# GaodeRender/triangle-splatting

Hardware: AMD Instinct MI355X
Metric: fwd+bwd Mpixels/sec @ 1M triangles, 1920x1080; achieved HBM GB/s (higher is better)
Workload: dtype f32

## Files before the change

triangle-splatting_amd/csrc/api.hip:

```cpp
#pragma GCC visibility push(default)
#include "../../include/ts2d.h"
#ifdef TS2D_LAB
#include "ts2d_lab.h"
#endif
#pragma GCC visibility pop
#include "ts2d_api.h"
#include <atomic>
#include <chrono>
#include <cstdarg>
#include <cstdio>
#include <cstring>
#include <mutex>
#include <string>
#include <vector>

namespace
{
thread_local std::string g_err;

struct ProfRow { std::string name; double ms = 0; int64_t launches = 0; };
struct ProfPending { int row; hipEvent_t a, b; };
std::mutex g_prof_mu;
bool g_prof_on = false;
std::string g_prof_only;
// ... 621 lines not shown
    case 8: src = g.tiles_touched; bytes = (size_t)P * 4; break;
    case 9:
    {
        std::vector<uint2> rc((size_t)P);
        if (dst_bytes < (size_t)P * 16) return ts_fail(TS2D_ERR_CAPACITY, "dst too small");
        if (P > 0)
        {
            TS_HIP(hipMemcpyAsync(rc.data(), g.rect, (size_t)P * sizeof(uint2), hipMemcpyDeviceToHost, s));
            TS_HIP(hipStreamSynchronize(s));
        }
        uint32_t *o = (uint32_t *)dst;
        for (int i = 0; i < P; i++)
        {
            o[4 * i] = rc[i].x & 0xffffu; o[4 * i + 1] = rc[i].x >> 16;
            o[4 * i + 2] = rc[i].y & 0xffffu; o[4 * i + 3] = rc[i].y >> 16;
        }
        return TS2D_OK;
    }
    case 10:
    {
        if (dst_bytes < (size_t)N * 8) return ts_fail(TS2D_ERR_CAPACITY, "dst too small");
        std::vector<uint32_t> tile((size_t)N), vals((size_t)N), depth((size_t)P);
        if (N > 0)
        {
            TS_HIP(hipMemcpyAsync(tile.data(), b.tile, (size_t)N * 4, hipMemcpyDeviceToHost, s));
            TS_HIP(hipMemcpyAsync(vals.data(), b.vals, (size_t)N * 4, hipMemcpyDeviceToHost, s));
            TS_HIP(hipMemcpyAsync(depth.data(), g.depth, (size_t)P * 4, hipMemcpyDeviceToHost, s));
            TS_HIP(hipStreamSynchronize(s));
        }
        uint64_t *o = (uint64_t *)dst;
        const uint32_t keymask = ts_tile_keymask(gx * gy);
        for (int64_t i = 0; i < N; i++) o[i] = ((uint64_t)(tile[i] & keymask) << 32) | depth[vals[i] & TS_ID_MASK];
        return TS2D_OK;
    }
    case 11: src = b.vals; bytes = (size_t)N * 4; break;
    case 12: src = im.ranges; bytes = (size_t)gx * gy * 8; break;
    case 13: src = im.n_contrib; bytes = (size_t)W * H * 4; break;
    case 14: src = im.final_T; bytes = (size_t)W * H * 4; break;
    case 15: src = b.k[(b.passes & 1) ^ 1]; bytes = (size_t)N * 4; break;
    case 16: src = b.v[(b.passes & 1) ^ 1]; bytes = (size_t)N * 4; break;
    case 17:
    {
        uint32_t top_const = 0;
        if (P > 0)
        {
            TS_HIP(hipMemcpyAsync(&top_const, g.top_const, 4, hipMemcpyDeviceToHost, s));
            TS_HIP(hipStreamSynchronize(s));
        }
        src = top_const ? g.sv[0] : g.sv[1];
        bytes = (size_t)P * 4;
        break;
    }
    case 18: src = g.rec; bytes = (size_t)P * TS_REC_FLOATS * 4; break;
    default: return ts_fail(TS2D_ERR_INVALID, "unknown field %d", field);
    }
    if (dst_bytes < bytes) return ts_fail(TS2D_ERR_CAPACITY, "dst too small");
    if (bytes)
    {
        TS_HIP(hipMemcpyAsync(dst, src, bytes, hipMemcpyDeviceToHost, s));
        TS_HIP(hipStreamSynchronize(s));
    }
    return TS2D_OK;
}

void ts2d_lab_force_ticket_passes(int on) { ts_force_ticket_passes(on != 0); }
void ts2d_lab_force_all_quadrants(int on) { g_lab_all_quadrants = on != 0; }
void ts2d_lab_force_kernel_cull(int on) { g_lab_kernel_cull = on != 0; }
void ts2d_lab_force_depth_pass4(int on) { ts_force_depth_pass4(on != 0); }
void ts2d_lab_depth_split(int mode, int bucket_cap) { ts_lab_depth_split(mode, bucket_cap); }
#endif

void ts2d_profile_enable(int on)
{
    std::lock_guard<std::mutex> lk(g_prof_mu);
    g_prof_on = on != 0;
}
void ts2d_profile_only(const char *name)
{
    std::lock_guard<std::mutex> lk(g_prof_mu);
    g_prof_only = name ? name : "";
}
void ts2d_profile_reset(void)
{
    std::lock_guard<std::mutex> lk(g_prof_mu);
    prof_drain();
    g_prof_rows.clear();
}
int ts2d_profile_read(int32_t index, char *name, size_t name_bytes, double *total_ms, int64_t *launches)
{
    std::lock_guard<std::mutex> lk(g_prof_mu);
    prof_drain();
    if (index < 0 || (size_t)index >= g_prof_rows.size()) return TS2D_ERR_INVALID;
    const ProfRow &r = g_prof_rows[index];
    if (name && name_bytes) { strncpy(name, r.name.c_str(), name_bytes - 1); name[name_bytes - 1] = 0; }
    if (total_ms) *total_ms = r.ms;
    if (launches) *launches = r.launches;
    return TS2D_OK;
}
}
```

triangle-splatting_amd/csrc/emit.hip:

```cpp
#include "ts2d_radix.h"
#include "ts2d_support.h"

namespace
{
constexpr uint32_t SMALL = 32;

#ifndef TS_EMIT_WAVES
#define TS_EMIT_WAVES 6
#endif
template <bool BM>
#if TS_EMIT_WAVES > 0
__global__ void __launch_bounds__(256, TS_EMIT_WAVES) scan_emit_kernel(
#else
__global__ void __launch_bounds__(256) scan_emit_kernel(
#endif
int P, int grid_x, int ntiles, GeometryStateView g, BinningStateView b, uint2 *ranges,
                                                         float *contrib_sum, float *contrib_max, long long capacity, int32_t *status, bool two_level,
                                                         QuadMaskArgs qmask)
{
    __shared__ uint32_t wtot[4];
    __shared__ unsigned long long wpart[4];
    const int t = threadIdx.x, lane = t & 63, wave = t >> 6;
    const int i = blockIdx.x * 256 + t;
    for (int k = i; k < ntiles; k += gridDim.x * 256) ranges[k] = make_uint2(0u, 0u);
    if (b.rs.tickets)
    {
        for (int k = i; k < b.rs.slabs + TS_RS_TICKET_EXTRA; k += gridDim.x * 256) b.rs.tickets[k] = 0u;
        for (int k = i; k < b.rs.slabs * NB; k += gridDim.x * 256) b.rs.slabacc[0][k] = 0u;
    }
    if (contrib_sum && i < P)
    {
        contrib_sum[i] = 0.0f;
        contrib_max[i] = 0.0f;
    }
    const bool valid = i < P;
    uint32_t tiles = valid ? g.tiles_sorted[i] : 0u;
    const uint32_t id_ahead = valid ? sorted_ids(g)[i] : 0u;
    const int sblock = blockIdx.x >> 2, quarter = blockIdx.x & 3;
    unsigned long long part = 0;
    if (two_level)
    {
        for (int k = t; k < (sblock >> 6); k += 256) part += g.supersum[k];
        if (t < (sblock & 63)) part += g.blocksum[(sblock & ~63) + t];
    }
    else
        for (int k = t; k < sblock; k += 256) part += g.blocksum[k];
    for (int q = 0; q < quarter; q++)
    {
        const int j = (sblock * 4 + q) * 256 + t;
        part += (j < P) ? g.tiles_sorted[j] : 0u;
    }
    if (capacity >= 0)
    {
        const unsigned long long live = g.blocksum[(P + SB - 1) / SB];
        const bool over = live > (unsigned long long)capacity;
        if (i == 0 && status) *status = over ? 1 : 0;
        if (over) tiles = 0u;
    }
    else if (i == 0 && status) *status = 0;
    const uint32_t inc = wave_inclusive_scan(tiles, lane);
    for (int o = 32; o > 0; o >>= 1) part += __shfl_xor(part, o);
    if (lane == 63) wtot[wave] = inc;
    if (lane == 0) wpart[wave] = part;
    __syncthreads();
    uint32_t before = 0;
    for (int w = 0; w < wave; w++) before += wtot[w];
    const unsigned long long qbase = wpart[0] + wpart[1] + wpart[2] + wpart[3];
    const uint32_t incl = (uint32_t)(qbase + before + inc);
    if (valid) g.offsets[i] = incl;
    const uint32_t id = tiles > 0 ? id_ahead : 0u;
    const uint32_t off = incl - tiles;
    uint2 rect = {0u, 0u};
    float4 rec0 = make_float4(0, 0, 0, 0), rec1 = rec0, rec2 = rec0;
    if (tiles > 0)
    {
        rect = g.rect[id];
        const float4 *rp = g.rec + 4 * (size_t)id;
        rec0 = rp[0];
        rec1 = rp[1];
        if (qmask.variant == 3) rec2 = rp[2];
    }
    const uint32_t minx = rect.x & 0xffffu, miny = rect.x >> 16, maxx = rect.y & 0xffffu, maxy = rect.y >> 16;
    uint32_t *tile_out = b.k[0], *val_out = b.v[0];
    constexpr bool qm = true;
    constexpr bool bm = BM;
    const float quad_g2 = qmask.g2;
    auto setup_from = [&](const float4 &r0, const float4 &r1, const float4 &r2, uint32_t tminx, uint32_t tminy, uint32_t tmaxx, uint32_t tmaxy) {
        if (qmask.variant == 0) return quad_setup_all();
        if (qmask.variant == 3)
        {
            const float E = quad_g2 == 2.0f ? support_scale<true>(1.0f, quad_g2) : support_scale<false>(1.0f, quad_g2);
            return quad_setup_3d(r0, r1, r2, E, qmask.tan_fovx, qmask.tan_fovy, qmask.W, qmask.H, qmask.inv_W, qmask.inv_H, (float)(tminx * TS_TILE) - 1.0f,
                                 (float)(tminy * TS_TILE) - 1.0f, (float)(tmaxx * TS_TILE), (float)(tmaxy * TS_TILE));
        }
        const float E = quad_g2 == 2.0f ? support_scale<true>(r1.z, quad_g2) : support_scale<false>(r1.z, quad_g2);
        return quad_setup<bm ? 3 : 7>(r0.x, r0.y, r0.z, r0.w, r1.x, r1.y, E);
    };
    auto setup_of = [&](uint32_t tri, uint32_t tminx, uint32_t tminy, uint32_t tmaxx, uint32_t tmaxy) {
        const float4 *rp = g.rec + 4 * (size_t)tri;
        return setup_from(rp[0], rp[1], qmask.variant == 3 ? rp[2] : make_float4(0, 0, 0, 0), tminx, tminy, tmaxx, tmaxy);
    };
    QuadSetup qs{};
    constexpr uint32_t STAGE = 2048;
    __shared__ uint32_t stage_t[STAGE];
    __shared__ __attribute__((aligned(16))) float4 region_b[256 * 4];
    uint32_t *const stage_v = (uint32_t *)region_b;
    const uint32_t run0 = (uint32_t)qbase, run = wtot[0] + wtot[1] + wtot[2] + wtot[3];
    const bool staged = run <= STAGE;
    const bool qstage = qm && staged;
    const uint32_t rw = maxx - minx, rh = maxy - miny;
    if (qm && tiles > 0)
    {
        qs = setup_from(rec0, rec1, rec2, minx, miny, maxx, maxy);
        if (qstage)
        {
            const QuadAffine qa = quad_anchor(qs, id, minx, miny, rw, rh);
            region_b[4 * t] = qa.a; region_b[4 * t + 1] = qa.b; region_b[4 * t + 2] = qa.c; region_b[4 * t + 3] = qa.d;
        }
    }
    if (tiles > 0 && tiles <= SMALL)
    {
        uint32_t o = off;
        if (staged)
        {
            o -= run0;
            for (uint32_t y = miny; y < maxy; y++)
                for (uint32_t x = minx; x < maxx; x++)
                {
                    stage_t[o] = qstage ? ((x - minx) | ((y - miny) << 12) | ((uint32_t)t << 24)) : y * grid_x + x;
                    if (!qstage) stage_v[o] = id;
                    o++;
                }
        }
        else
            for (uint32_t y = miny; y < maxy; y++)
                for (uint32_t x = minx; x < maxx; x++)
                {
                    if (bm)
                    {
                        const uint32_t m16 = block_mask(qs, (float)(x * TS_TILE), (float)(y * TS_TILE));
                        tile_out[o] = (y * grid_x + x) | (m16 << 16);
                        val_out[o] = id | (quadrants_of_blocks(m16) << TS_ID_BITS);
                    }
                    else
                    {
                        tile_out[o] = y * grid_x + x;
                        val_out[o] = qm ? id | (quadrant_mask(qs, (float)(x * TS_TILE), (float)(y * TS_TILE)) << TS_ID_BITS) : id;
                    }
                    o++;
                }
    }
    unsigned long long big = ballot64(tiles > SMALL);
    while (big)
    {
        const int j = __builtin_ctzll(big);
        big &= big - 1;
        const uint32_t t_minx = __shfl(minx, j), t_miny = __shfl(miny, j), t_maxx = __shfl(maxx, j), t_maxy = __shfl(maxy, j);
        const uint32_t t_tiles = __shfl(tiles, j), t_off = __shfl(off, j), t_id = __shfl(id, j);
        const uint32_t w = t_maxx - t_minx;
        QuadSetup tq{};
        if (qm && !staged) tq = setup_of(t_id, t_minx, t_miny, t_maxx, t_maxy);
        for (uint32_t k = lane; k < t_tiles; k += 64)
        {
            const uint32_t y = t_miny + k / w, x = t_minx + k % w;
            if (staged)
            {
                stage_t[t_off - run0 + k] = qstage ? ((k % w) | ((k / w) << 12) | ((uint32_t)(wave * 64 + j) << 24)) : y * grid_x + x;
                if (!qstage) stage_v[t_off - run0 + k] = t_id;
            }
            else
            {
                if (bm)
                {
                    const uint32_t m16 = block_mask(tq, (float)(x * TS_TILE), (float)(y * TS_TILE));
                    tile_out[t_off + k] = (y * grid_x + x) | (m16 << 16);
                    val_out[t_off + k] = t_id | (quadrants_of_blocks(m16) << TS_ID_BITS);
                }
                else
                {
                    tile_out[t_off + k] = y * grid_x + x;
                    val_out[t_off + k] = qm ? t_id | (quadrant_mask(tq, (float)(x * TS_TILE), (float)(y * TS_TILE)) << TS_ID_BITS) : t_id;
                }
            }
        }
    }
    if (staged)
    {
        __syncthreads();
        for (uint32_t k = t; k < run; k += 256)
        {
            uint32_t tl = stage_t[k], v;
            if (qstage)
            {
                const uint32_t dx = tl & 0xfffu, dy = (tl >> 12) & 0xfffu, slot = tl >> 24;
                QuadAffine qa;
                qa.a = region_b[4 * slot]; qa.b = region_b[4 * slot + 1]; qa.c = region_b[4 * slot + 2]; qa.d = region_b[4 * slot + 3];
                const uint32_t org = __float_as_uint(qa.d.z), x = (org & 0xffffu) + dx, y = (org >> 16) + dy;
                if (bm)
                {
                    const uint32_t m16 = block_mask_affine(qa, dx, dy, x, y);
                    v = __float_as_uint(qa.d.y) | (quadrants_of_blocks(m16) << TS_ID_BITS);
                    tl = (y * grid_x + x) | (m16 << 16);
                }
                else
                {
                    v = __float_as_uint(qa.d.y) | (quadrant_mask_affine(qa, dx, dy, x, y) << TS_ID_BITS);
                    tl = y * grid_x + x;
                }
            }
            else v = stage_v[k];
            tile_out[run0 + k] = tl;
            val_out[run0 + k] = v;
        }
    }
}

__global__ void __launch_bounds__(256) tile_ranges_kernel(int64_t N, const unsigned long long *n_dev, const uint32_t *__restrict__ tile,
                                                           uint2 *__restrict__ ranges, uint32_t keymask)
{
    const int64_t i0 = ((int64_t)blockIdx.x * 256 + threadIdx.x) * 4;
    if (n_dev)
    {
        const unsigned long long live = *n_dev;
        N = (live <= (unsigned long long)N) ? (int64_t)live : 0;
    }
    if (i0 >= N) return;
    uint32_t k[4];
    if (i0 + 3 < N)
    {
        const uint4 q = *(const uint4 *)(tile + i0);
        k[0] = q.x & keymask; k[1] = q.y & keymask; k[2] = q.z & keymask; k[3] = q.w & keymask;
    }
    else
        for (int j = 0; j < 4; j++) k[j] = i0 + j < N ? tile[i0 + j] & keymask : 0u;
    uint32_t prev = i0 > 0 ? tile[i0 - 1] & keymask : 0u;
#pragma unroll
    for (int j = 0; j < 4; j++)
    {
        const int64_t i = i0 + j;
        if (i >= N) break;
        const uint32_t cur = k[j];
        if (i == 0) ranges[cur].x = 0;
        else if (cur != prev)
        {
            ranges[prev].y = (uint32_t)i;
            ranges[cur].x = (uint32_t)i;
        }
        if (i == N - 1) ranges[cur].y = (uint32_t)N;
        prev = cur;
    }
}
}

void ts_launch_emit_keys(int P, int grid_x, int ntiles, const GeometryStateView &g, const BinningStateView &b, const ImageStateView &im,
                         float *contrib_sum, float *contrib_max, int64_t capacity, int32_t *status, const QuadMaskArgs &qmask, hipStream_t s)
{
    if (P <= 0) return;
    const dim3 grid((unsigned)(((P + SB - 1) / SB) * 4));
    if (qmask.blocks)
        hipLaunchKernelGGL(scan_emit_kernel<true>, grid, dim3(256), 0, s, P, grid_x, ntiles, g, b, im.ranges, contrib_sum, contrib_max, (long long)capacity,
                           status, ts_scan_two_level(P), qmask);
    else
        hipLaunchKernelGGL(scan_emit_kernel<false>, grid, dim3(256), 0, s, P, grid_x, ntiles, g, b, im.ranges, contrib_sum, contrib_max, (long long)capacity,
                           status, ts_scan_two_level(P), qmask);
}
const unsigned long long *ts_instance_count_dev(const GeometryStateView &g, int P) { return (const unsigned long long *)(g.blocksum + (P + SB - 1) / SB); }

void ts_launch_tile_ranges(int64_t N, const unsigned long long *n_dev, int ntiles, const BinningStateView &b, const ImageStateView &im, hipStream_t s)
{
    if (N <= 0) return;
    hipLaunchKernelGGL(tile_ranges_kernel, dim3((unsigned)((N + 1023) / 1024)), dim3(256), 0, s, N, n_dev, b.tile, im.ranges, ts_tile_keymask(ntiles));
}
```

triangle-splatting_amd/csrc/mesh_preprocess.hip:

```cpp
#include "ts2d_common.h"
#include "ts2d_math.h"
#include "ts2d_preprocess_launch.h"

using namespace ts;

namespace
{
constexpr float BOX_MARGIN = 2e-3f;

__global__ void __launch_bounds__(256) mesh_preprocess_kernel(MeshArgs a, GeometryStateView g)
{
    const int f = blockIdx.x * 256 + threadIdx.x;
    clear_tickets(g, f, a.F);
    if (f >= a.F) return;
    uint32_t out_tiles = 0;
    uint2 out_rect = {0u, 0u};
    float out_key = 0.0f;
    float rec[TS_REC_FLOATS];
#pragma unroll
    for (int i = 0; i < TS_REC_FLOATS; i++) rec[i] = 0.0f;

    int32_t i1 = a.faces[3 * (size_t)f], i2 = a.faces[3 * (size_t)f + 1], i3 = a.faces[3 * (size_t)f + 2];
    if (i1 > i2) { const int32_t t = i1; i1 = i2; i2 = t; }
    if (i2 > i3) { const int32_t t = i2; i2 = i3; i3 = t; }
    if (i1 > i2) { const int32_t t = i1; i1 = i2; i2 = t; }
    do
    {
        if ((uint32_t)i1 >= (uint32_t)a.V || (uint32_t)i2 >= (uint32_t)a.V || (uint32_t)i3 >= (uint32_t)a.V) break;
        const float *p1 = a.vertices + 3 * (size_t)i1, *p2 = a.vertices + 3 * (size_t)i2, *p3 = a.vertices + 3 * (size_t)i3;
        const f3 v1 = xform_point_4x3({p1[0], p1[1], p1[2]}, a.viewmatrix), v2 = xform_point_4x3({p2[0], p2[1], p2[2]}, a.viewmatrix),
                 v3 = xform_point_4x3({p3[0], p3[1], p3[2]}, a.viewmatrix);
        if (!(v1.z > a.znear && v2.z > a.znear && v3.z > a.znear)) break;

        const float hw = (float)a.W * 0.5f, hh = (float)a.H * 0.5f;
        const f2 s1 = {(v1.x / (v1.z * a.tan_fovx) + 1.0f) * hw, (v1.y / (v1.z * a.tan_fovy) + 1.0f) * hh};
        const f2 s2 = {(v2.x / (v2.z * a.tan_fovx) + 1.0f) * hw, (v2.y / (v2.z * a.tan_fovy) + 1.0f) * hh};
        const f2 s3 = {(v3.x / (v3.z * a.tan_fovx) + 1.0f) * hw, (v3.y / (v3.z * a.tan_fovy) + 1.0f) * hh};
        const float area2 = cross(sub(s2, s1), sub(s3, s1));
        if (!(fabsf(area2) > 0.0f)) break;

        const float xmin = fminf(fminf(s1.x, s2.x), s3.x), xmax = fmaxf(fmaxf(s1.x, s2.x), s3.x);
        const float ymin = fminf(fminf(s1.y, s2.y), s3.y), ymax = fmaxf(fmaxf(s1.y, s2.y), s3.y);
        if (!(xmax >= 0.0f && xmin <= (float)a.W && ymax >= 0.0f && ymin <= (float)a.H)) break;
        const int px0 = max(0, f2i(ceilf(fmaxf(xmin, 0.0f) - 0.5f - BOX_MARGIN))), px1 = min(a.W - 1, f2i(floorf(fminf(xmax, (float)a.W) - 0.5f + BOX_MARGIN)));
        const int py0 = max(0, f2i(ceilf(fmaxf(ymin, 0.0f) - 0.5f - BOX_MARGIN))), py1 = min(a.H - 1, f2i(floorf(fminf(ymax, (float)a.H) - 0.5f + BOX_MARGIN)));
        if (px1 < px0 || py1 < py0) break;
        const int rminx = px0 / TS_TILE, rminy = py0 / TS_TILE, rmaxx = px1 / TS_TILE + 1, rmaxy = py1 / TS_TILE + 1;

        const f3 n = cross(sub(v2, v1), sub(v3, v1));
        rec[0] = s1.x; rec[1] = s1.y; rec[2] = s2.x; rec[3] = s2.y; rec[4] = s3.x; rec[5] = s3.y;
        rec[6] = n.x; rec[7] = n.y; rec[8] = n.z;
        rec[9] = dot(n, v1);
        rec[10] = fminf(fminf(v1.z, v2.z), v3.z);
        rec[11] = fmaxf(fmaxf(v1.z, v2.z), v3.z);
        out_key = rec[10];
        out_tiles = (uint32_t)(rmaxx - rminx) * (uint32_t)(rmaxy - rminy);
        out_rect = {(uint32_t)rminx | ((uint32_t)rminy << 16), (uint32_t)rmaxx | ((uint32_t)rmaxy << 16)};
    } while (false);

    g.tiles_touched[f] = out_tiles;
    g.rect[f] = out_rect;
    g.depth[f] = out_key;
    float4 *r = g.rec + 4 * (size_t)f;
    r[0] = make_float4(rec[0], rec[1], rec[2], rec[3]);
    r[1] = make_float4(rec[4], rec[5], rec[6], rec[7]);
    r[2] = make_float4(rec[8], rec[9], rec[10], rec[11]);
    r[3] = make_float4(rec[12], rec[13], rec[14], rec[15]);
}
}

void ts_launch_mesh_preprocess(const MeshArgs &a, const GeometryStateView &g, hipStream_t s)
{
    if (a.F <= 0) return;
    hipLaunchKernelGGL(mesh_preprocess_kernel, dim3((unsigned)((a.F + 255) / 256)), dim3(256), 0, s, a, g);
}
```

triangle-splatting_amd/csrc/preprocess.hip:

```cpp
#include "ts2d_common.h"
#include "ts2d_math.h"
#include "ts2d_sh.h"
#include "ts2d_preprocess_launch.h"

using namespace ts;

namespace
{
__device__ __forceinline__ void preprocess_fwd_one(const PreprocessArgs &a, int32_t *__restrict__ radii, const GeometryStateView &g,
                                                   int idx, const float *vp, const float *shp, float4 *rec_row)
{
    int out_radius = 0;
    uint32_t out_tiles = 0;
    uint2 out_rect = {0u, 0u};
    uint8_t out_clamped = 0;
    float out_depth = 0.0f;
    float rec[TS_REC_FLOATS];
#pragma unroll
    for (int i = 0; i < TS_REC_FLOATS; i++) rec[i] = 0.0f;

    const f3 v1 = {vp[0], vp[1], vp[2]}, v2 = {vp[3], vp[4], vp[5]}, v3 = {vp[6], vp[7], vp[8]};
    const f3 center = divf(add(add(v1, v2), v3), 3.0f);
    const f3 center_proj = project_point(center, a.projmatrix);

// ... 30 lines not shown
        if (a.back_culling) { if (area2 >= -TS_EPS) break; }
        else { if (fabsf(area2) < TS_EPS) break; }

        const float dilation = 3.0f;
        const f2 d1 = add(center_2D, scale(dilation, r1_2D));
        const f2 d2 = add(center_2D, scale(dilation, r2_2D));
        const f2 d3 = add(center_2D, scale(dilation, r3_2D));
        const f2 v_min = {fminf(fminf(d1.x, d2.x), d3.x), fminf(fminf(d1.y, d2.y), d3.y)};
        const f2 v_max = {fmaxf(fmaxf(d1.x, d2.x), d3.x), fmaxf(fmaxf(d1.y, d2.y), d3.y)};

        const int rminx = min(a.grid_x, max(0, f2i(v_min.x / TS_TILE)));
        const int rminy = min(a.grid_y, max(0, f2i(v_min.y / TS_TILE)));
        const int rmaxx = min(a.grid_x, max(0, f2i((v_max.x + TS_TILE - 1) / TS_TILE)));
        const int rmaxy = min(a.grid_y, max(0, f2i((v_max.y + TS_TILE - 1) / TS_TILE)));
        if (rmaxx <= rminx || rmaxy <= rminy) break;

        {
        f3 rgb = {0, 0, 0};
        if (a.use_shs)
        {
            const f3 cp = {a.campos[0], a.campos[1], a.campos[2]};
            rgb = sh_to_rgb(a.D, shp, center, cp);
            out_clamped = (uint8_t)((rgb.x < 0 ? 1 : 0) | (rgb.y < 0 ? 2 : 0) | (rgb.z < 0 ? 4 : 0));
            rgb = {fmaxf(rgb.x, 0.0f), fmaxf(rgb.y, 0.0f), fmaxf(rgb.z, 0.0f)};
        }
        else
        {
            const float *fp = a.feature + (size_t)idx * a.C;
            rgb.x = a.C > 0 ? fp[0] : 0.0f;
            rgb.y = a.C > 1 ? fp[1] : 0.0f;
            rgb.z = a.C > 2 ? fp[2] : 0.0f;
        }
        rec[0] = v1_2D.x; rec[1] = v1_2D.y; rec[2] = v2_2D.x; rec[3] = v2_2D.y; rec[4] = v3_2D.x; rec[5] = v3_2D.y;
        rec[6] = a.opacity[idx];
        rec[7] = rgb.x; rec[8] = rgb.y; rec[9] = rgb.z;
        if (a.rich_info)
        {
            f3 n_view = cross(r1_view, r2_view);
            n_view = divf(n_view, norm(n_view));
            rec[10] = n_view.x; rec[11] = n_view.y; rec[12] = n_view.z;
            rec[13] = r1_view.z + center_view.z; rec[14] = r2_view.z + center_view.z; rec[15] = r3_view.z + center_view.z;
        }
        }
        out_depth = center_view.z;
        out_tiles = (uint32_t)(rmaxx - rminx) * (uint32_t)(rmaxy - rminy);
        out_rect = {(uint32_t)rminx | ((uint32_t)rminy << 16), (uint32_t)rmaxx | ((uint32_t)rmaxy << 16)};
        out_radius = f2i(fmaxf(ceilf((v_max.x - v_min.x) * 0.5f), ceilf((v_max.y - v_min.y) * 0.5f)));
    } while (false);

    {
        radii[idx] = out_radius;
        g.tiles_touched[idx] = out_tiles;
        g.rect[idx] = out_rect;
        g.depth[idx] = out_depth;
        g.clamped[idx] = out_clamped;
        float4 *r = rec_row;
        r[0] = make_float4(rec[0], rec[1], rec[2], rec[3]);
        r[1] = make_float4(rec[4], rec[5], rec[6], rec[7]);
        r[2] = make_float4(rec[8], rec[9], rec[10], rec[11]);
        r[3] = make_float4(rec[12], rec[13], rec[14], rec[15]);
    }
}

__device__ __forceinline__ void project_vec_approx_bwd(f3 p, f3 v, float tx, float ty, f2 dL_dvec_proj, f3 &dL_dp, f3 &dL_dv)
{
    const float px_pz = p.x / p.z, py_pz = p.y / p.z;
    const float vx_pz = v.x / p.z, vy_pz = v.y / p.z, vz_pz = v.z / p.z;
    const f2 d = {dL_dvec_proj.x / (p.z * tx), dL_dvec_proj.y / (p.z * ty)};
    dL_dv = {d.x, d.y, -d.x * px_pz - d.y * py_pz};
    dL_dp = {-d.x * vz_pz, -d.y * vz_pz, d.x * (2.0f * vz_pz * px_pz - vx_pz) + d.y * (2.0f * vz_pz * py_pz - vy_pz)};
}

__device__ __forceinline__ void preprocess_bwd_one(const PreprocessArgs &a, const int32_t *__restrict__ radii,
                                                   const GeometryStateView &g, const float *__restrict__ grad_rec, int idx,
                                                   const float *vp, const float *shp, float *ov, float *osh,
                                                   float *__restrict__ dL_dcenter2D, float *__restrict__ dL_dfeature,
                                                   float *__restrict__ dL_dopacity)
{
    float *oc = dL_dcenter2D + 2 * (size_t)idx;
    if (radii[idx] <= 0)
    {
#pragma unroll
        for (int i = 0; i < 9; i++) ov[i] = 0.0f;
        oc[0] = 0.0f; oc[1] = 0.0f;
        dL_dopacity[idx] = 0.0f;
        for (int c = 0; c < a.C; c++) dL_dfeature[(size_t)idx * a.C + c] = 0.0f;
        if (a.use_shs && osh)
        {
#pragma unroll
            for (int k = 0; k < 48; k++)
                if (k < a.M * 3) osh[k] = 0.0f;
        }
        return;
    }

    const float4 *gr = (const float4 *)(grad_rec + TS_GRAD_FLOATS * (size_t)idx);
    const float4 g0 = gr[0], g1 = gr[1], g2 = gr[2], g3 = gr[3];
    const f2 dL_dv1_2D = {g0.x, g0.y}, dL_dv2_2D = {g0.z, g0.w}, dL_dv3_2D = {g1.x, g1.y};
    const float dL_dop = g1.z;
    f3 dL_drgb = {g1.w, g2.x, g2.y};
    const f3 dL_dnormal_view = {g2.z, g2.w, g3.x};
    const f3 dL_dv_depth = {g3.y, g3.z, g3.w};

    const f3 v1 = {vp[0], vp[1], vp[2]}, v2 = {vp[3], vp[4], vp[5]}, v3 = {vp[6], vp[7], vp[8]};
    const f3 center = divf(add(add(v1, v2), v3), 3.0f);
    const f3 center_view = xform_point_4x3(center, a.viewmatrix);
// ... 102 lines not shown
```

triangle-splatting_amd/csrc/preprocess3d.hip:

```cpp
#include "ts2d_common.h"
#include "ts2d_math.h"
#include "ts2d_sh.h"
#include "ts2d_preprocess_launch.h"

using namespace ts;

namespace
{
__device__ __forceinline__ float proj_to_pix(float v, int S) { return (v + 1.0f) * S * 0.5f - 0.5f; }

__device__ __forceinline__ void preprocess3d_fwd_one(const PreprocessArgs &a, int32_t *__restrict__ radii, const GeometryStateView &g,
                                                     int idx, const float *vp, const float *shp, float4 *rec_row)
{
    int out_radius = 0;
    uint32_t out_tiles = 0;
    uint2 out_rect = {0u, 0u};
    uint8_t out_clamped = 0;
    float out_depth = 0.0f;
    float rec[TS_REC_FLOATS];
#pragma unroll
    for (int i = 0; i < TS_REC_FLOATS; i++) rec[i] = 0.0f;

    const f3 v1 = {vp[0], vp[1], vp[2]}, v2 = {vp[3], vp[4], vp[5]}, v3 = {vp[6], vp[7], vp[8]};
    do
// ... 5 lines not shown
        if (norm(normal_view) < TS_EPS) break;
        if (a.back_culling && normal_view.z >= 0) break;

        const float dilation = 3.0f;
        const f3 center = divf(add(add(v1, v2), v3), 3.0f);
        const f3 d1 = add(center, scale(dilation, sub(v1, center)));
        const f3 d2 = add(center, scale(dilation, sub(v2, center)));
        const f3 d3 = add(center, scale(dilation, sub(v3, center)));
        const f3 p1 = project_point(d1, a.projmatrix), p2 = project_point(d2, a.projmatrix), p3 = project_point(d3, a.projmatrix);
        if (p1.z <= 0 || p2.z <= 0 || p3.z <= 0) break;

        const f2 q1 = {proj_to_pix(p1.x, a.W), proj_to_pix(p1.y, a.H)};
        const f2 q2 = {proj_to_pix(p2.x, a.W), proj_to_pix(p2.y, a.H)};
        const f2 q3 = {proj_to_pix(p3.x, a.W), proj_to_pix(p3.y, a.H)};
        const f2 v_min = {fminf(fminf(q1.x, q2.x), q3.x), fminf(fminf(q1.y, q2.y), q3.y)};
        const f2 v_max = {fmaxf(fmaxf(q1.x, q2.x), q3.x), fmaxf(fmaxf(q1.y, q2.y), q3.y)};
        const int rminx = min(a.grid_x, max(0, f2i(v_min.x / TS_TILE)));
        const int rminy = min(a.grid_y, max(0, f2i(v_min.y / TS_TILE)));
        const int rmaxx = min(a.grid_x, max(0, f2i((v_max.x + TS_TILE - 1) / TS_TILE)));
        const int rmaxy = min(a.grid_y, max(0, f2i((v_max.y + TS_TILE - 1) / TS_TILE)));
        if (rmaxx <= rminx || rmaxy <= rminy) break;

        f3 rgb = {0, 0, 0};
        if (a.use_shs)
        {
            const f3 cp = {a.campos[0], a.campos[1], a.campos[2]};
            rgb = sh_to_rgb(a.D, shp, center, cp);
            out_clamped = (uint8_t)((rgb.x < 0 ? 1 : 0) | (rgb.y < 0 ? 2 : 0) | (rgb.z < 0 ? 4 : 0));
            rgb = {fmaxf(rgb.x, 0.0f), fmaxf(rgb.y, 0.0f), fmaxf(rgb.z, 0.0f)};
        }
        else
        {
            const float *fp = a.feature + (size_t)idx * a.C;
            rgb.x = a.C > 0 ? fp[0] : 0.0f;
            rgb.y = a.C > 1 ? fp[1] : 0.0f;
            rgb.z = a.C > 2 ? fp[2] : 0.0f;
        }
        rec[0] = v1_view.x; rec[1] = v1_view.y; rec[2] = v1_view.z;
        rec[3] = v2_view.x; rec[4] = v2_view.y; rec[5] = v2_view.z;
        rec[6] = v3_view.x; rec[7] = v3_view.y; rec[8] = v3_view.z;
        rec[9] = normal_view.x; rec[10] = normal_view.y; rec[11] = normal_view.z;
        rec[12] = a.opacity[idx];
        rec[13] = rgb.x; rec[14] = rgb.y; rec[15] = rgb.z;
        out_depth = center_view.z;
        out_tiles = (uint32_t)(rmaxx - rminx) * (uint32_t)(rmaxy - rminy);
        out_rect = {(uint32_t)rminx | ((uint32_t)rminy << 16), (uint32_t)rmaxx | ((uint32_t)rmaxy << 16)};
        out_radius = f2i(fmaxf(ceilf((v_max.x - v_min.x) * 0.5f), ceilf((v_max.y - v_min.y) * 0.5f)));
    } while (false);

    {
        radii[idx] = out_radius;
        g.tiles_touched[idx] = out_tiles;
        g.rect[idx] = out_rect;
        g.depth[idx] = out_depth;
        g.clamped[idx] = out_clamped;
        float4 *r = rec_row;
        r[0] = make_float4(rec[0], rec[1], rec[2], rec[3]);
        r[1] = make_float4(rec[4], rec[5], rec[6], rec[7]);
        r[2] = make_float4(rec[8], rec[9], rec[10], rec[11]);
        r[3] = make_float4(rec[12], rec[13], rec[14], rec[15]);
    }
}

__device__ __forceinline__ void preprocess3d_bwd_one(const PreprocessArgs &a, const int32_t *__restrict__ radii,
                                                     const GeometryStateView &g, const float *__restrict__ grad_rec, int idx,
                                                     const float *vp, const float *shp, float *ov, float *osh,
                                                     float *__restrict__ dL_dcenter2D, float *__restrict__ dL_dfeature,
                                                     float *__restrict__ dL_dopacity)
{
    float *oc = dL_dcenter2D + 2 * (size_t)idx;
    if (radii[idx] <= 0)
    {
#pragma unroll
        for (int i = 0; i < 9; i++) ov[i] = 0.0f;
        oc[0] = 0.0f; oc[1] = 0.0f;
        dL_dopacity[idx] = 0.0f;
        for (int c = 0; c < a.C; c++) dL_dfeature[(size_t)idx * a.C + c] = 0.0f;
        if (a.use_shs && osh)
        {
#pragma unroll
            for (int k = 0; k < 48; k++)
                if (k < a.M * 3) osh[k] = 0.0f;
        }
        return;
    }
    const f3 v1 = {vp[0], vp[1], vp[2]}, v2 = {vp[3], vp[4], vp[5]}, v3 = {vp[6], vp[7], vp[8]};
    const float4 *rp = g.rec + 4 * (size_t)idx;
    const float4 r0 = rp[0], r1 = rp[1], r2 = rp[2];
    const f3 v1_view = {r0.x, r0.y, r0.z}, v2_view = {r0.w, r1.x, r1.y}, v3_view = {r1.z, r1.w, r2.x};
    const float4 *gr = (const float4 *)(grad_rec + TS_GRAD_FLOATS * (size_t)idx);
    const float4 g0 = gr[0], g1 = gr[1], g2 = gr[2], g3 = gr[3];
    f3 gv1 = {g0.x, g0.y, g0.z}, gv2 = {g0.w, g1.x, g1.y}, gv3 = {g1.z, g1.w, g2.x};
    const f3 gn = {g2.y, g2.z, g2.w};
    const float gop = g3.x;
    const f3 grgb = {g3.y, g3.z, g3.w};
    f3 grgb_out = grgb;

    gv1 = add(gv1, cross(sub(v2_view, v3_view), gn));
    gv2 = add(gv2, cross(sub(v3_view, v1_view), gn));
    gv3 = add(gv3, cross(sub(v1_view, v2_view), gn));
    f3 dL_dv1 = xform_vec_4x3_T(gv1, a.viewmatrix), dL_dv2 = xform_vec_4x3_T(gv2, a.viewmatrix),
       dL_dv3 = xform_vec_4x3_T(gv3, a.viewmatrix);
    if (a.use_shs)
    {
        const f3 center = divf(add(add(v1, v2), v3), 3.0f);
        const uint8_t cl = g.clamped[idx];
// ... 41 lines not shown
```

triangle-splatting_amd/csrc/ts2d_common.h:

```cpp
#pragma once
#include <hip/hip_runtime.h>
#include <stddef.h>
#include <stdint.h>

#define TS_TILE 16
#define TS_ALIGN 256

#define TS_REC_FLOATS 16

#define TS_ID_BITS 28
#define TS_ID_MASK 0x0FFFFFFFu
#define TS_GRAD_FLOATS 16

#ifndef TS_RS_CHUNK
#define TS_RS_CHUNK 4096
#endif
#define TS_RS_CHUNK_MID 2048
#define TS_RS_CHUNK_SMALL 1024
#define TS_RS_SMALL_BELOW 2500000
static inline int ts_instance_chunk(size_t n) { return n <= (size_t)TS_RS_SMALL_BELOW ? TS_RS_CHUNK_SMALL : TS_RS_CHUNK; }
static inline int ts_depth_chunk(size_t n) { return n <= (size_t)TS_RS_SMALL_BELOW ? TS_RS_CHUNK_SMALL : TS_RS_CHUNK_MID; }
#define TS_RS_BINS 256
#define TS_RS_TICKET_EXTRA 8
struct RadixScratchView
{
    uint32_t *table;
    uint32_t *slabtot;
    uint32_t *binbase;
    uint32_t *tickets;
    uint32_t *slabacc[2];
    int chunks, slabs;
    int chunk;
};

struct GeometryStateView
{
    float4 *rec;
    float *depth;
    uint32_t *tiles_touched;
    uint2 *rect;
    uint8_t *clamped;
    uint32_t *sk[2], *sv[2];
    uint32_t *depth_sorted;
    uint32_t *perm;
    uint32_t *top_const;
    uint32_t *tiles_sorted;
    uint32_t *offsets;
    uint64_t *blocksum;
    uint64_t *supersum;
    RadixScratchView rs;
};

struct BinningStateView
{
    uint32_t *k[2], *v[2];
    uint32_t *tile;
    uint32_t *vals;
    int passes;
    RadixScratchView rs;
};

struct ImageStateView
{
    uint2 *ranges;
    uint32_t *n_contrib;
    float *final_T;
    int32_t *status;
};

static inline size_t ts_align_up(size_t v) { return (v + TS_ALIGN - 1) & ~(size_t)(TS_ALIGN - 1); }

template <typename T>
static inline void ts_carve(char *&p, T *&out, size_t count)
{
    p = (char *)ts_align_up((size_t)p);
    out = (T *)p;
    p += count * sizeof(T);
}

static inline void ts_carve_radix(char *&p, size_t n, RadixScratchView &r, int chunk = TS_RS_CHUNK, int reserve_chunk = 0)
{
    r.chunk = chunk;
    r.chunks = (int)((n + chunk - 1) / chunk);
    r.slabs = (r.chunks + 63) / 64;
    const int rc = reserve_chunk > 0 ? reserve_chunk : chunk;
    const size_t chunks = (n + rc - 1) / rc, slabs = (chunks + 63) / 64;
    ts_carve(p, r.table, chunks * TS_RS_BINS);
    ts_carve(p, r.slabtot, slabs * TS_RS_BINS);
    ts_carve(p, r.binbase, (size_t)TS_RS_BINS);
    ts_carve(p, r.tickets, slabs + TS_RS_TICKET_EXTRA);
    ts_carve(p, r.slabacc[0], slabs * TS_RS_BINS);
    ts_carve(p, r.slabacc[1], slabs * TS_RS_BINS);
}

static inline size_t ts_carve_geometry(char *base, int32_t P, GeometryStateView &v)
{
    char *p = base;
    size_t n = (size_t)(P > 0 ? P : 0);
    ts_carve(p, v.rec, n * 4);
    ts_carve(p, v.depth, n);
    ts_carve(p, v.tiles_touched, n);
    ts_carve(p, v.rect, n);
    ts_carve(p, v.clamped, n);
    ts_carve(p, v.sk[0], n);
    ts_carve(p, v.sk[1], n);
    ts_carve(p, v.sv[0], n);
    ts_carve(p, v.sv[1], n);
    v.depth_sorted = v.sk[1];
    v.perm = v.sv[1];
    ts_carve(p, v.tiles_sorted, n);
    ts_carve(p, v.offsets, n);
    ts_carve(p, v.blocksum, (n + 1023) / 1024 + 2);
    ts_carve(p, v.supersum, ((n + 1023) / 1024 + 63) / 64 + 1);
    ts_carve_radix(p, n, v.rs, ts_depth_chunk(n));
    v.top_const = v.rs.tickets + v.rs.slabs + 4;
    return (size_t)(p - base) + TS_ALIGN;
}

static inline int ts_higher_msb(uint32_t n)
{
    uint32_t msb = sizeof(n) * 4, step = msb;
    while (step > 1)
    {
        step /= 2;
        if (n >> msb) msb += step;
        else msb -= step;
    }
    if (n >> msb) msb++;
    return (int)msb;
}

static inline int ts_tile_bits(int ntiles) { return ts_higher_msb((uint32_t)(ntiles > 1 ? ntiles - 1 : 1)); }
#define TS_BLOCKMASK_MAX_TILES 65535
static inline uint32_t ts_tile_keymask(int ntiles) { return ntiles <= TS_BLOCKMASK_MAX_TILES ? 0xFFFFu : 0xFFFFFFFFu; }

static inline size_t ts_carve_binning(char *base, int64_t N, int32_t W, int32_t H, BinningStateView &v)
{
    char *p = base;
    size_t n = (size_t)(N > 0 ? N : 0);
    int gx = (W + TS_TILE - 1) / TS_TILE, gy = (H + TS_TILE - 1) / TS_TILE;
    ts_carve(p, v.k[0], n);
    ts_carve(p, v.k[1], n);
    ts_carve(p, v.v[0], n);
    ts_carve(p, v.v[1], n);
    v.passes = (ts_tile_bits(gx * gy) + 7) / 8;
    v.tile = v.k[v.passes & 1];
    v.vals = v.v[v.passes & 1];
    ts_carve_radix(p, n, v.rs, ts_instance_chunk(n), TS_RS_CHUNK_SMALL);
    return (size_t)(p - base) + TS_ALIGN;
}

static inline int64_t ts_binning_capacity(size_t bytes, int32_t W, int32_t H)
{
    BinningStateView v;
    if (bytes < ts_carve_binning(nullptr, 0, W, H, v)) return -1;
// ... 178 lines not shown
```

Measured before the change: 1359.

## Restructure scan-emit to single-wave blocks with ordered chunks and packed rects

The scan/emit kernel moves from 256-thread blocks to 64-thread single-wave blocks. Block order comes from an ordered-chunk helper, which removes the block-level __syncthreads and LDS reductions. Prefix sums now use buffer loads with out-of-range protection, and the tail of the in-superblock prefix is loaded with vectorized b128 loads. A packed 32-bit rect (rect4) is written in preprocess and read in emit instead of the 8-byte rect, with a fallback when the rect does not fit in 8 bits per field. The risks are that the LDS staging capacity per block shrinks, which sends more work down the unstaged path, and that preprocess now does an extra global write.

```diff
diff --git a/triangle-splatting_amd/csrc/api.hip b/triangle-splatting_amd/csrc/api.hip
--- a/triangle-splatting_amd/csrc/api.hip
+++ b/triangle-splatting_amd/csrc/api.hip
@@ -697,6 +697,7 @@
         break;
     }
     case 18: src = g.rec; bytes = (size_t)P * TS_REC_FLOATS * 4; break;
+    case 19: src = g.rect4; bytes = (size_t)P * 4; break;
     default: return ts_fail(TS2D_ERR_INVALID, "unknown field %d", field);
     }
     if (dst_bytes < bytes) return ts_fail(TS2D_ERR_CAPACITY, "dst too small");
diff --git a/triangle-splatting_amd/csrc/emit.hip b/triangle-splatting_amd/csrc/emit.hip
--- a/triangle-splatting_amd/csrc/emit.hip
+++ b/triangle-splatting_amd/csrc/emit.hip
@@ -4,30 +4,51 @@
 namespace
 {
 constexpr uint32_t SMALL = 32;
+constexpr int UNIT = 64;
+constexpr uint32_t TS_EMIT_STAGE = 512;
 
 #ifndef TS_EMIT_WAVES
-#define TS_EMIT_WAVES 6
+#define TS_EMIT_WAVES 5
 #endif
+typedef uint32_t u32x2 __attribute__((ext_vector_type(2)));
+typedef uint32_t u32x4 __attribute__((ext_vector_type(4)));
+template <int G>
+__device__ __forceinline__ unsigned long long front_sum64(const uint64_t *p, int n, int lane)
+{
+    const __amdgpu_buffer_rsrc_t r = __builtin_amdgcn_make_buffer_rsrc((void *)p, 0, n * 8, 0x00020000);
+    unsigned long long s = 0;
+    for (int c = 0; c < n; c += UNIT * G)
+    {
+#pragma unroll
+        for (int j = 0; j < G; j++)
+        {
+            const u32x2 v = __builtin_amdgcn_raw_buffer_load_b64(r, (c + lane + UNIT * j) * 8, 0, 0);
+            s += (unsigned long long)v.x | ((unsigned long long)v.y << 32);
+        }
+    }
+    return s;
+}
 template <bool BM>
 #if TS_EMIT_WAVES > 0
-__global__ void __launch_bounds__(256, TS_EMIT_WAVES) scan_emit_kernel(
+__global__ void __launch_bounds__(UNIT, TS_EMIT_WAVES) scan_emit_kernel(
 #else
-__global__ void __launch_bounds__(256) scan_emit_kernel(
+__global__ void __launch_bounds__(UNIT) scan_emit_kernel(
 #endif
 int P, int grid_x, int ntiles, GeometryStateView g, BinningStateView b, uint2 *ranges,
                                                          float *contrib_sum, float *contrib_max, long long capacity, int32_t *status, bool two_level,
                                                          QuadMaskArgs qmask)
 {
-    __shared__ uint32_t wtot[4];
-    __shared__ unsigned long long wpart[4];
-    const int t = threadIdx.x, lane = t & 63, wave = t >> 6;
-    const int i = blockIdx.x * 256 + t;
-    for (int k = i; k < ntiles; k += gridDim.x * 256) ranges[k] = make_uint2(0u, 0u);
+    const int lane = threadIdx.x;
+    const int gi = blockIdx.x * UNIT + lane, gn = gridDim.x * UNIT;
+    for (int k = gi; k < ntiles; k += gn) ranges[k] = make_uint2(0u, 0u);
     if (b.rs.tickets)
     {
-        for (int k = i; k < b.rs.slabs + TS_RS_TICKET_EXTRA; k += gridDim.x * 256) b.rs.tickets[k] = 0u;
-        for (int k = i; k < b.rs.slabs * NB; k += gridDim.x * 256) b.rs.slabacc[0][k] = 0u;
-    }
+        for (int k = gi; k < b.rs.slabs + TS_RS_TICKET_EXTRA; k += gn) b.rs.tickets[k] = 0u;
+        for (int k = gi; k < b.rs.slabs * NB; k += gn) b.rs.slabacc[0][k] = 0u;
+    }
+    const int unit = rs_chunk_of_block((P + UNIT - 1) / UNIT);
+    if (unit < 0) return;
+    const int i = unit * UNIT + lane;
     if (contrib_sum && i < P)
     {
         contrib_sum[i] = 0.0f;
@@ -36,20 +57,18 @@
     const bool valid = i < P;
     uint32_t tiles = valid ? g.tiles_sorted[i] : 0u;
     const uint32_t id_ahead = valid ? sorted_ids(g)[i] : 0u;
-    const int sblock = blockIdx.x >> 2, quarter = blockIdx.x & 3;
-    unsigned long long part = 0;
-    if (two_level)
-    {
-        for (int k = t; k < (sblock >> 6); k += 256) part += g.supersum[k];
-        if (t < (sblock & 63)) part += g.blocksum[(sblock & ~63) + t];
-    }
-    else
-        for (int k = t; k < sblock; k += 256) part += g.blocksum[k];
-    for (int q = 0; q < quarter; q++)
-    {
-        const int j = (sblock * 4 + q) * 256 + t;
-        part += (j < P) ? g.tiles_sorted[j] : 0u;
-    }
+    const int sblock = unit / (SB / UNIT), sub = unit % (SB / UNIT);
+    u32x4 early[SB / UNIT / 4];
+    {
+        const __amdgpu_buffer_rsrc_t r = __builtin_amdgcn_make_buffer_rsrc((void *)(g.tiles_sorted + (size_t)sblock * SB), 0, sub * UNIT * 4, 0x00020000);
+#pragma unroll
+        for (int k = 0; k < SB / UNIT / 4; k++) early[k] = __builtin_amdgcn_raw_buffer_load_b128(r, (lane + UNIT * k) * 16, 0, 0);
+    }
+    unsigned long long part;
+    if (two_level) part = front_sum64<1>(g.supersum, sblock >> 6, lane) + front_sum64<1>(g.blocksum + (sblock & ~63), sblock & 63, lane);
+    else part = front_sum64<8>(g.blocksum, sblock, lane);
+#pragma unroll
+    for (int k = 0; k < SB / UNIT / 4; k++) part += (early[k].x + early[k].y) + (early[k].z + early[k].w);
     if (capacity >= 0)
     {
         const unsigned long long live = g.blocksum[(P + SB - 1) / SB];
@@ -59,30 +78,31 @@
     }
     else if (i == 0 && status) *status = 0;
     const uint32_t inc = wave_inclusive_scan(tiles, lane);
-    for (int o = 32; o > 0; o >>= 1) part += __shfl_xor(part, o);
-    if (lane == 63) wtot[wave] = inc;
-    if (lane == 0) wpart[wave] = part;
-    __syncthreads();
-    uint32_t before = 0;
-    for (int w = 0; w < wave; w++) before += wtot[w];
-    const unsigned long long qbase = wpart[0] + wpart[1] + wpart[2] + wpart[3];
-    const uint32_t incl = (uint32_t)(qbase + before + inc);
+    const uint32_t run0 = (uint32_t)wave_sum64(part), run = (uint32_t)__shfl((int)inc, UNIT - 1);
+    const uint32_t incl = run0 + inc;
     if (valid) g.offsets[i] = incl;
     const uint32_t id = tiles > 0 ? id_ahead : 0u;
     const uint32_t off = incl - tiles;
-    uint2 rect = {0u, 0u};
+    uint32_t minx = 0u, miny = 0u, maxx = 0u, maxy = 0u;
     float4 rec0 = make_float4(0, 0, 0, 0), rec1 = rec0, rec2 = rec0;
     if (tiles > 0)
     {
-        rect = g.rect[id];
+        const uint32_t r4 = g.rect4[id];
         const float4 *rp = g.rec + 4 * (size_t)id;
         rec0 = rp[0];
         rec1 = rp[1];
         if (qmask.variant == 3) rec2 = rp[2];
-    }
-    const uint32_t minx = rect.x & 0xffffu, miny = rect.x >> 16, maxx = rect.y & 0xffffu, maxy = rect.y >> 16;
+        if (r4 == TS_RECT4_NONE)
+        {
+            const uint2 rect = g.rect[id];
+            minx = rect.x & 0xffffu; miny = rect.x >> 16; maxx = rect.y & 0xffffu; maxy = rect.y >> 16;
+        }
+        else
+        {
+            minx = r4 & 0xffu; miny = (r4 >> 8) & 0xffu; maxx = minx + ((r4 >> 16) & 0xffu); maxy = miny + (r4 >> 24);
+        }
+    }
     uint32_t *tile_out = b.k[0], *val_out = b.v[0];
-    constexpr bool qm = true;
     constexpr bool bm = BM;
     const float quad_g2 = qmask.g2;
     auto setup_from = [&](const float4 &r0, const float4 &r1, const float4 &r2, uint32_t tminx, uint32_t tminy, uint32_t tmaxx, uint32_t tmaxy) {
@@ -100,22 +120,30 @@
         const float4 *rp = g.rec + 4 * (size_t)tri;
         return setup_from(rp[0], rp[1], qmask.variant == 3 ? rp[2] : make_float4(0, 0, 0, 0), tminx, tminy, tmaxx, tmaxy);
     };
+    auto put = [&](const QuadSetup &q, uint32_t o, uint32_t tri, uint32_t x, uint32_t y) {
+        if (bm)
+        {
+            const uint32_t m16 = block_mask(q, (float)(x * TS_TILE), (float)(y * TS_TILE));
+            tile_out[o] = (y * grid_x + x) | (m16 << 16);
+            val_out[o] = tri | (quadrants_of_blocks(m16) << TS_ID_BITS);
+        }
+        else
+        {
+            tile_out[o] = y * grid_x + x;
+            val_out[o] = tri | (quadrant_mask(q, (float)(x * TS_TILE), (float)(y * TS_TILE)) << TS_ID_BITS);
+        }
+    };
+    __shared__ uint32_t stage_t[TS_EMIT_STAGE];
+    __shared__ __attribute__((aligned(16))) float4 anchor[UNIT * 4];
+    const bool staged = run <= TS_EMIT_STAGE;
     QuadSetup qs{};
-    constexpr uint32_t STAGE = 2048;
-    __shared__ uint32_t stage_t[STAGE];
-    __shared__ __attribute__((aligned(16))) float4 region_b[256 * 4];
-    uint32_t *const stage_v = (uint32_t *)region_b;
-    const uint32_t run0 = (uint32_t)qbase, run = wtot[0] + wtot[1] + wtot[2] + wtot[3];
-    const bool staged = run <= STAGE;
-    const bool qstage = qm && staged;
-    const uint32_t rw = maxx - minx, rh = maxy - miny;
-    if (qm && tiles > 0)
+    if (tiles > 0)
     {
         qs = setup_from(rec0, rec1, rec2, minx, miny, maxx, maxy);
-        if (qstage)
-        {
-            const QuadAffine qa = quad_anchor(qs, id, minx, miny, rw, rh);
-            region_b[4 * t] = qa.a; region_b[4 * t + 1] = qa.b; region_b[4 * t + 2] = qa.c; region_b[4 * t + 3] = qa.d;
+        if (staged)
+        {
+            const QuadAffine qa = quad_anchor(qs, id, minx, miny, maxx - minx, maxy - miny);
+            anchor[4 * lane] = qa.a; anchor[4 * lane + 1] = qa.b; anchor[4 * lane + 2] = qa.c; anchor[4 * lane + 3] = qa.d;
         }
     }
     if (tiles > 0 && tiles <= SMALL)
@@ -125,30 +153,11 @@
         {
             o -= run0;
             for (uint32_t y = miny; y < maxy; y++)
-                for (uint32_t x = minx; x < maxx; x++)
-                {
-                    stage_t[o] = qstage ? ((x - minx) | ((y - miny) << 12) | ((uint32_t)t << 24)) : y * grid_x + x;
-                    if (!qstage) stage_v[o] = id;
-                    o++;
-                }
+                for (uint32_t x = minx; x < maxx; x++) stage_t[o++] = (x - minx) | ((y - miny) << 12) | ((uint32_t)lane << 24);
         }
         else
             for (uint32_t y = miny; y < maxy; y++)
-                for (uint32_t x = minx; x < maxx; x++)
-                {
-                    if (bm)
-                    {
-                        const uint32_t m16 = block_mask(qs, (float)(x * TS_TILE), (float)(y * TS_TILE));
-                        tile_out[o] = (y * grid_x + x) | (m16 << 16);
-                        val_out[o] = id | (quadrants_of_blocks(m16) << TS_ID_BITS);
-                    }
-                    else
-                    {
-                        tile_out[o] = y * grid_x + x;
-                        val_out[o] = qm ? id | (quadrant_mask(qs, (float)(x * TS_TILE), (float)(y * TS_TILE)) << TS_ID_BITS) : id;
-                    }
-                    o++;
-                }
+                for (uint32_t x = minx; x < maxx; x++) put(qs, o++, id, x, y);
     }
     unsigned long long big = ballot64(tiles > SMALL);
     while (big)
@@ -159,56 +168,34 @@
         const uint32_t t_tiles = __shfl(tiles, j), t_off = __shfl(off, j), t_id = __shfl(id, j);
         const uint32_t w = t_maxx - t_minx;
         QuadSetup tq{};
-        if (qm && !staged) tq = setup_of(t_id, t_minx, t_miny, t_maxx, t_maxy);
-        for (uint32_t k = lane; k < t_tiles; k += 64)
-        {
-            const uint32_t y = t_miny + k / w, x = t_minx + k % w;
-            if (staged)
+        if (!staged) tq = setup_of(t_id, t_minx, t_miny, t_maxx, t_maxy);
+        for (uint32_t k = lane; k < t_tiles; k += UNIT)
+        {
+            if (staged) stage_t[t_off - run0 + k] = (k % w) | ((k / w) << 12) | ((uint32_t)j << 24);
+            else put(tq, t_off + k, t_id, t_minx + k % w, t_miny + k / w);
+        }
+    }
+    if (staged)
+    {
+        wave_lds_order();
+        for (uint32_t k = lane; k < run; k += UNIT)
+        {
+            uint32_t tl = stage_t[k], v;
+            const uint32_t dx = tl & 0xfffu, dy = (tl >> 12) & 0xfffu, slot = tl >> 24;
+            QuadAffine qa;
+            qa.a = anchor[4 * slot]; qa.b = anchor[4 * slot + 1]; qa.c = anchor[4 * slot + 2]; qa.d = anchor[4 * slot + 3];
+            const uint32_t org = __float_as_uint(qa.d.z), x = (org & 0xffffu) + dx, y = (org >> 16) + dy;
+            if (bm)
             {
-                stage_t[t_off - run0 + k] = qstage ? ((k % w) | ((k / w) << 12) | ((uint32_t)(wave * 64 + j) << 24)) : y * grid_x + x;
-                if (!qstage) stage_v[t_off - run0 + k] = t_id;
+                const uint32_t m16 = block_mask_affine(qa, dx, dy, x, y);
+                v = __float_as_uint(qa.d.y) | (quadrants_of_blocks(m16) << TS_ID_BITS);
+                tl = (y * grid_x + x) | (m16 << 16);
             }
             else
             {
-                if (bm)
-                {
-                    const uint32_t m16 = block_mask(tq, (float)(x * TS_TILE), (float)(y * TS_TILE));
-                    tile_out[t_off + k] = (y * grid_x + x) | (m16 << 16);
-                    val_out[t_off + k] = t_id | (quadrants_of_blocks(m16) << TS_ID_BITS);
-                }
-                else
-                {
-                    tile_out[t_off + k] = y * grid_x + x;
-                    val_out[t_off + k] = qm ? t_id | (quadrant_mask(tq, (float)(x * TS_TILE), (float)(y * TS_TILE)) << TS_ID_BITS) : t_id;
-                }
+                v = __float_as_uint(qa.d.y) | (quadrant_mask_affine(qa, dx, dy, x, y) << TS_ID_BITS);
+                tl = y * grid_x + x;
             }
-        }
-    }
-    if (staged)
-    {
-        __syncthreads();
-        for (uint32_t k = t; k < run; k += 256)
-        {
-            uint32_t tl = stage_t[k], v;
-            if (qstage)
-            {
-                const uint32_t dx = tl & 0xfffu, dy = (tl >> 12) & 0xfffu, slot = tl >> 24;
-                QuadAffine qa;
-                qa.a = region_b[4 * slot]; qa.b = region_b[4 * slot + 1]; qa.c = region_b[4 * slot + 2]; qa.d = region_b[4 * slot + 3];
-                const uint32_t org = __float_as_uint(qa.d.z), x = (org & 0xffffu) + dx, y = (org >> 16) + dy;
-                if (bm)
-                {
-                    const uint32_t m16 = block_mask_affine(qa, dx, dy, x, y);
-                    v = __float_as_uint(qa.d.y) | (quadrants_of_blocks(m16) << TS_ID_BITS);
-                    tl = (y * grid_x + x) | (m16 << 16);
-                }
-                else
-                {
-                    v = __float_as_uint(qa.d.y) | (quadrant_mask_affine(qa, dx, dy, x, y) << TS_ID_BITS);
-                    tl = y * grid_x + x;
-                }
-            }
-            else v = stage_v[k];
             tile_out[run0 + k] = tl;
             val_out[run0 + k] = v;
         }
@@ -256,12 +243,12 @@
                          float *contrib_sum, float *contrib_max, int64_t capacity, int32_t *status, const QuadMaskArgs &qmask, hipStream_t s)
 {
     if (P <= 0) return;
-    const dim3 grid((unsigned)(((P + SB - 1) / SB) * 4));
+    const dim3 grid((unsigned)(8 * (((P + UNIT - 1) / UNIT + 7) / 8)));
     if (qmask.blocks)
-        hipLaunchKernelGGL(scan_emit_kernel<true>, grid, dim3(256), 0, s, P, grid_x, ntiles, g, b, im.ranges, contrib_sum, contrib_max, (long long)capacity,
+        hipLaunchKernelGGL(scan_emit_kernel<true>, grid, dim3(UNIT), 0, s, P, grid_x, ntiles, g, b, im.ranges, contrib_sum, contrib_max, (long long)capacity,
                            status, ts_scan_two_level(P), qmask);
     else
-        hipLaunchKernelGGL(scan_emit_kernel<false>, grid, dim3(256), 0, s, P, grid_x, ntiles, g, b, im.ranges, contrib_sum, contrib_max, (long long)capacity,
+        hipLaunchKernelGGL(scan_emit_kernel<false>, grid, dim3(UNIT), 0, s, P, grid_x, ntiles, g, b, im.ranges, contrib_sum, contrib_max, (long long)capacity,
                            status, ts_scan_two_level(P), qmask);
 }
 const unsigned long long *ts_instance_count_dev(const GeometryStateView &g, int P) { return (const unsigned long long *)(g.blocksum + (P + SB - 1) / SB); }
diff --git a/triangle-splatting_amd/csrc/mesh_preprocess.hip b/triangle-splatting_amd/csrc/mesh_preprocess.hip
--- a/triangle-splatting_amd/csrc/mesh_preprocess.hip
+++ b/triangle-splatting_amd/csrc/mesh_preprocess.hip
@@ -60,6 +60,7 @@
 
     g.tiles_touched[f] = out_tiles;
     g.rect[f] = out_rect;
+    g.rect4[f] = ts_pack_rect4(out_rect);
     g.depth[f] = out_key;
     float4 *r = g.rec + 4 * (size_t)f;
     r[0] = make_float4(rec[0], rec[1], rec[2], rec[3]);
diff --git a/triangle-splatting_amd/csrc/preprocess.hip b/triangle-splatting_amd/csrc/preprocess.hip
--- a/triangle-splatting_amd/csrc/preprocess.hip
+++ b/triangle-splatting_amd/csrc/preprocess.hip
@@ -106,6 +106,7 @@
         radii[idx] = out_radius;
         g.tiles_touched[idx] = out_tiles;
         g.rect[idx] = out_rect;
+        g.rect4[idx] = ts_pack_rect4(out_rect);
         g.depth[idx] = out_depth;
         g.clamped[idx] = out_clamped;
         float4 *r = rec_row;
diff --git a/triangle-splatting_amd/csrc/preprocess3d.hip b/triangle-splatting_amd/csrc/preprocess3d.hip
--- a/triangle-splatting_amd/csrc/preprocess3d.hip
+++ b/triangle-splatting_amd/csrc/preprocess3d.hip
@@ -81,6 +81,7 @@
         radii[idx] = out_radius;
         g.tiles_touched[idx] = out_tiles;
         g.rect[idx] = out_rect;
+        g.rect4[idx] = ts_pack_rect4(out_rect);
         g.depth[idx] = out_depth;
         g.clamped[idx] = out_clamped;
         float4 *r = rec_row;
diff --git a/triangle-splatting_amd/csrc/ts2d_common.h b/triangle-splatting_amd/csrc/ts2d_common.h
--- a/triangle-splatting_amd/csrc/ts2d_common.h
+++ b/triangle-splatting_amd/csrc/ts2d_common.h
@@ -39,6 +39,7 @@
     float *depth;
     uint32_t *tiles_touched;
     uint2 *rect;
+    uint32_t *rect4;
     uint8_t *clamped;
     uint32_t *sk[2], *sv[2];
     uint32_t *depth_sorted;
@@ -67,6 +68,14 @@
     float *final_T;
     int32_t *status;
 };
+
+#define TS_RECT4_NONE 0xFFFFFFFFu
+static __host__ __device__ inline uint32_t ts_pack_rect4(uint2 rect)
+{
+    const uint32_t minx = rect.x & 0xffffu, miny = rect.x >> 16, w = (rect.y & 0xffffu) - minx, h = (rect.y >> 16) - miny;
+    const bool fits = minx < 255u && miny < 255u && w < 255u && h < 255u;
+    return fits ? minx | (miny << 8) | (w << 16) | (h << 24) : TS_RECT4_NONE;
+}
 
 static inline size_t ts_align_up(size_t v) { return (v + TS_ALIGN - 1) & ~(size_t)(TS_ALIGN - 1); }
 
@@ -101,6 +110,7 @@
     ts_carve(p, v.depth, n);
     ts_carve(p, v.tiles_touched, n);
     ts_carve(p, v.rect, n);
+    ts_carve(p, v.rect4, n);
     ts_carve(p, v.clamped, n);
     ts_carve(p, v.sk[0], n);
     ts_carve(p, v.sk[1], n);
```

After: 1355. Within noise of the previous version (-0.3%).
